# roatienza/efficientspeech

Measured on AMD Instinct MI355X. Metric: mel-frames/sec (whole node), full Phoneme2Mel forward, higher is better.
Workload: dtype f32 (weight GEMMs: fp32 operands split into 2 f16 pieces (22 significand bits, weights pre-scaled 2^8), 3 f16-MFMA products, fp32 accumulate)

## Files before the change

efficientspeech_amd/csrc/enc_block16.h:

```cpp
#pragma once
#include "chain16.h"
#include "enc_attn_ffn.h"

namespace esmi {

struct B016Lds {
    static constexpr int C = 32, LD = C + 4, NK = 128, LDX = NK + 4;
    static constexpr int xP = 0;
    static constexpr int xT = xP + 128 * LD;
    static constexpr int y1P = xT + C * LDX;
    static constexpr int priv = y1P + 130 * LD;
    static constexpr int priv_sz = 2 * 16 * LD;
    static constexpr int par = priv + 8 * priv_sz;
    static constexpr int wts = par + 512;
    static constexpr int total = wts + 24 * 256;
};
static_assert(B016Lds::total * 4 <= 160 * 1024, "enc_b0_16: LDS");
enum { B0_PROJB = 0, B0_LN1G = 32, B0_LN1B = 64, B0_FFNB = 96, B0_FFNB0 = 128, B0_FFNB2 = 160, B0_MLP2B = 192, B0_LN2G = 224, B0_LN2B = 256 };

template <int NKT>
__device__ __forceinline__ void enc_b0_16_body(const EncAttnFfnP& p) {
    using namespace c16;
    typedef B016Lds M;
    constexpr int C = M::C, LD = M::LD, LDX = M::LDX;
    ESMI_DYN_LDS(lds);
    ESMI_CT_INIT(0);
    ESMI_CT();
    const int nw = (int)(blockDim.x >> 6), w = uniform_i(wave_id());
    const int lane = lane_id(), i = lane & 15, g = lane >> 4;
    const int b = (int)blockIdx.x, rot = b;
    const int pos = 16 * w + i;
    unsigned* const ldu = reinterpret_cast<unsigned*>(lds);
    unsigned* const xP = ldu + M::xP;
    unsigned* const xT = ldu + M::xT;
    unsigned* const y1P = ldu + M::y1P;
    float* const xf = lds + M::priv + w * M::priv_sz;
    unsigned* const qP = ldu + M::priv + w * M::priv_sz + 16 * LD;
    float* const par = lds + M::par;
    float* const wM = lds + M::wts, * const wO = wM + 4 * 256, * const wF = wO + 4 * 256, * const w2 = wF + 12 * 256;
    const int wp = wpos(lane), lw1 = wlane(lane, 1);
    const f32x4 z4 = zero4();
    const int* idb = p.m.ids + (long)b * p.m.n_in;
    int id[3];
#pragma unroll
    for (int j = 0; j < 3; ++j) {
        const int ti = pos + j - 1;
        const bool ok = ti >= 0 && ti < p.m.n_in;
        const int v = idb[ok ? ti : 0];
        id[j] = !ok ? -1 : ((v < 0 || v >= p.m.vocab) ? 0 : v);
    }
    dma_frags(p.m.qkv_w, wM, 4, w, nw, lane, rot);
    dma_frags(p.proj_w, wO, 4, w, nw, lane, rot);
    dma_frags(p.ffn_w, wF, 12, w, nw, lane, rot);
    dma_frags(p.mlp2_w, w2, 4, w, nw, lane, rot);
    {
        const int v8 = lane >> 3, c8 = 4 * (lane & 7);
        auto pick8 = [&](const float* a0, const float* a1, const float* a2, const float* a3, const float* a4, const float* a5, const float* a6,
                         const float* a7) __attribute__((always_inline)) {
            const float* lo = v8 & 1 ? (v8 & 2 ? a3 : a1) : (v8 & 2 ? a2 : a0);
            const float* hi = v8 & 1 ? (v8 & 2 ? a7 : a5) : (v8 & 2 ? a6 : a4);
            return (v8 & 4 ? hi : lo) + c8;
        };
        if (w == 0 % nw) lds_dma16(pick8(p.proj_b, p.ln1_g, p.ln1_b, p.ffn_b, p.ffn_b0, p.ffn_b2, p.mlp2_b, p.ln2_g), par, lane);
        if (w == 1 % nw) lds_dma16(p.ln2_b + c8, par + B0_LN2B, lane);
    }
    if (w == 0 && lane < LD) {
        y1P[lane] = 0u;
        y1P[(16 * nw + 1) * LD + lane] = 0u;
    }
    if (nw < NKT) {
        for (int e = (int)threadIdx.x; e < C * LDX; e += (int)blockDim.x) xT[e] = 0u;
        for (int e = (int)threadIdx.x + 16 * nw * LD; e < 16 * NKT * LD; e += (int)blockDim.x) xP[e] = 0u;
        wg_sync_lds();
    }
    const bool rout = pos >= p.N;
    unsigned mb = 0;
    {
        const BufRsrc r_mask = make_rsrc(p.mask ? p.mask + (long)b * p.mask_len : nullptr, p.mask_len);
        for (int q = 0; q < p.mask_pool; ++q) {
            const int idx = pos * p.mask_pool + q;
            mb |= buf_ld_u8(r_mask, (unsigned)idx) | (unsigned)(p.mask && idx >= p.mask_len);
        }
    }
    const bool rz = !rout && mb != 0;
    ESMI_CT();
    f32x4 xacc[2] = {z4, z4};
#pragma unroll
    for (int j = 0; j < 3; ++j) {
        const float* row = p.m.emb_conv + ((long)j * p.m.vocab + (id[j] < 0 ? 0 : id[j])) * C + 4 * g;
#pragma unroll
        for (int nt = 0; nt < 2; ++nt) {
            const f32x4 v = ld4(row + 16 * nt);
            if (id[j] >= 0) xacc[nt] += v;
        }
    }
    if (rout) { xacc[0] = z4; xacc[1] = z4; }
#pragma unroll
    for (int nt = 0; nt < 2; ++nt) {
        planes_store(xP + pos * LD + wp, nt, C / 2, xacc[nt]);
        *reinterpret_cast<f32x4*>(xf + i * LD + 16 * nt + 4 * g) = xacc[nt];
    }
    lds_wave_sync();
#pragma unroll
    for (int ct = 0; ct < 2; ++ct) {
        f32x4 v;
#pragma unroll
        for (int r = 0; r < 4; ++r) v[r] = xf[(4 * g + r) * LD + 16 * ct + i];
        unsigned h1a, h2a, h1b, h2b;
        split_f16_pair(v[0], v[1], h1a, h2a);
        split_f16_pair(v[2], v[3], h1b, h2b);
        unsigned* dst = xT + (16 * ct + i) * LDX + 16 * (w >> 1) + 4 * g + 2 * (w & 1);
        *reinterpret_cast<u32x2*>(dst) = u32x2{h1a, h1b};
        *reinterpret_cast<u32x2*>(dst + M::NK / 2) = u32x2{h2a, h2b};
    }
    ESMI_CT();
    wait_vm0();
    wg_sync_lds();
    ESMI_CT();
    {
        f32x4 q[2] = {z4, z4};
        const unsigned* rowp = xP + pos * LD + 4 * g;
        gemm_pf<2, 1, 1>(q, wM, lw1, 0, [&](int) __attribute__((always_inline)) { return planes_load(rowp, 0, C / 2); });
#pragma unroll
        for (int nt = 0; nt < 2; ++nt) planes_store(qP + i * LD + wp, nt, C / 2, q[nt] * kF16WScaleInv);
        lds_wave_sync();
    }
    f32x4 s[NKT];
    {
        const f16x2p qf = planes_load(qP + i * LD + 4 * g, 0, C / 2);
        f16x2p kf[NKT];
#pragma unroll
        for (int kt = 0; kt < NKT; ++kt) kf[kt] = planes_load(xP + (16 * kt + i) * LD + 4 * g, 0, C / 2);
        sched_fence();
#pragma unroll
        for (int kt = 0; kt < NKT; ++kt) s[kt] = mfma16_f16(kf[kt].h2, qf.h1, z4);
#pragma unroll
        for (int kt = 0; kt < NKT; ++kt) s[kt] = mfma16_f16(kf[kt].h1, qf.h2, s[kt]);
#pragma unroll
        for (int kt = 0; kt < NKT; ++kt) s[kt] = mfma16_f16(kf[kt].h1, qf.h1, s[kt]);
    }
    ESMI_CT();
    float mx = -INFINITY;
#pragma unroll
    for (int kt = 0; kt < NKT; ++kt) {
#pragma unroll
        for (int r = 0; r < 4; ++r) {
            const int key = 16 * kt + 4 * g + r;
            const float v = key < p.N ? s[kt][r] * p.scale : -INFINITY;
            s[kt][r] = v;
            mx = fmaxf(mx, v);
        }
    }
    mx = row_max4(mx);
    float den = 0.0f;
#pragma unroll
    for (int kt = 0; kt < NKT; ++kt) {
#pragma unroll
        for (int r = 0; r < 4; ++r) {
            const float e = exp_fast_f32(s[kt][r] - mx);
            s[kt][r] = e;
            den += e;
        }
    }
    const float inv = rcp_fast_f32(row_sum4(den));
    ESMI_CT();
    f32x4 o[2] = {z4, z4};
    {
        f16x2p vf[NKT / 2][2];
#pragma unroll
        for (int ks = 0; ks < NKT / 2; ++ks) {
#pragma unroll
            for (int ct = 0; ct < 2; ++ct) {
                const unsigned* vp = xT + (16 * ct + i) * LDX + 16 * ks + 4 * g;
                vf[ks][ct].h1 = *reinterpret_cast<const u32x4*>(vp);
                vf[ks][ct].h2 = *reinterpret_cast<const u32x4*>(vp + M::NK / 2);
            }
        }
        sched_fence();
#pragma unroll
        for (int ks = 0; ks < NKT / 2; ++ks) {
            const f16x2p pf = split_f16x2(s[2 * ks] * inv, s[2 * ks + 1] * inv);
#pragma unroll
            for (int ct = 0; ct < 2; ++ct) o[ct] = mfma16_f16(vf[ks][ct].h2, pf.h1, o[ct]);
#pragma unroll
            for (int ct = 0; ct < 2; ++ct) o[ct] = mfma16_f16(vf[ks][ct].h1, pf.h2, o[ct]);
#pragma unroll
            for (int ct = 0; ct < 2; ++ct) o[ct] = mfma16_f16(vf[ks][ct].h1, pf.h1, o[ct]);
        }
    }
    ESMI_CT();
#pragma unroll
    for (int nt = 0; nt < 2; ++nt) planes_store(qP + i * LD + wp, nt, C / 2, o[nt]);
    lds_wave_sync();
    f32x4 y[2] = {z4, z4};
    {
        const unsigned* rowp = qP + i * LD + 4 * g;
        gemm_pf<2, 1, 1>(y, wO, lw1, 0, [&](int) __attribute__((always_inline)) { return planes_load(rowp, 0, C / 2); });
        f32x4 gg[2], bb[2];
#pragma unroll
        for (int nt = 0; nt < 2; ++nt) {
// ... 56 lines not shown
    }
    ESMI_CT();
}

template <int NKT>
__global__ __launch_bounds__(64 * 8, 2) void enc_b0_16_kernel(const EncAttnFfnP p) {
    enc_b0_16_body<NKT>(p);
}

struct B116Lds {
    static constexpr int C = 64, LD = C + 4, CIN = 32, NK = 64, LDX = NK + 4, LDC = 2 * C + 4;
    static constexpr int r1 = 0;
    static constexpr int r2 = r1 + 66 * LD;
    static constexpr int r3 = r2 + 64 * LD;
    static constexpr int r3_sz = 8 * 16 * LD;
    static constexpr int stats = r3 + r3_sz;
    static constexpr int par = stats + 256;
    static constexpr int wY = par + 768;
    static constexpr int wX = wY + 48 * 256;
    static constexpr int total = wX + 32 * 256;
};
static_assert(64 * B116Lds::LDC <= B116Lds::r3_sz && B116Lds::total * 4 <= 160 * 1024, "enc_b1_16: LDS");
enum { B1_PROJB = 0, B1_LN1G = 64, B1_LN1B = 128, B1_FFNB = 192, B1_FFNB0 = 256, B1_FFNB2 = 320, B1_MLP2B = 384, B1_LN2G = 448, B1_LN2B = 512 };

__device__ __forceinline__ void layernorm_pair16(f32x4 (&v)[2], const f32x4 (&gg)[2], const f32x4 (&bb)[2], float* st, int c, int i, int g,
                                                 float eps = 1e-5f) {
    using namespace c16;
    float s = (v[0][0] + v[0][1]) + (v[0][2] + v[0][3]) + ((v[1][0] + v[1][1]) + (v[1][2] + v[1][3]));
    const float mean_l = row_sum4(s) * (1.0f / 32.0f);
    float q = 0.0f;
#pragma unroll
    for (int nt = 0; nt < 2; ++nt) {
#pragma unroll
        for (int e = 0; e < 4; ++e) {
            const float d = v[nt][e] - mean_l;
            q = fmaf(d, d, q);
        }
    }
    const float m2_l = row_sum4(q);
    if (g == 0) *reinterpret_cast<f32x2*>(st + (c * 16 + i) * 2) = f32x2{mean_l, m2_l};
    wg_sync_lds();
    const f32x2 o = *reinterpret_cast<const f32x2*>(st + ((c ^ 1) * 16 + i) * 2);
    const float ma = c == 0 ? mean_l : o[0], mb = c == 0 ? o[0] : mean_l;
    const float qa = c == 0 ? m2_l : o[1], qb = c == 0 ? o[1] : m2_l;
    const float mean = 0.5f * (ma + mb);
    const float d = mb - ma;
    const float m2 = (qa + qb) + d * d * 16.0f;
    const float rstd = rsqrt_fast_f32(m2 * (1.0f / 64.0f) + eps);
#pragma unroll
    for (int nt = 0; nt < 2; ++nt) {
#pragma unroll
        for (int e = 0; e < 4; ++e) v[nt][e] = fmaf((v[nt][e] - mean) * rstd, gg[nt][e], bb[nt][e]);
    }
}

__device__ __forceinline__ void enc_b1_16_body(const EncAttnFfnP& p) {
    using namespace c16;
    typedef B116Lds M;
    constexpr int C = M::C, LD = M::LD, LDX = M::LDX, LDC = M::LDC, CIN = M::CIN, NKT = 4;
    ESMI_DYN_LDS(lds);
    ESMI_CT_INIT(1);
    ESMI_CT();
    const int nw = (int)(blockDim.x >> 6), w = uniform_i(wave_id());
    const int nrt = nw >> 1, rt = w >> 1, c = w & 1;
    const int lane = lane_id(), i = lane & 15, g = lane >> 4;
    const int b = (int)blockIdx.x, rot = b;
    const int pos = 16 * rt + i;
    unsigned* const ldu = reinterpret_cast<unsigned*>(lds);
    unsigned* const xP = ldu + M::r1;
    unsigned* const y1P = ldu + M::r1;
    unsigned* const xT = ldu + M::r2;
    unsigned* const hidP = ldu + M::r2;
    float* const xf = lds + M::r3 + w * (16 * LD);
    unsigned* const qP = ldu + M::r3 + w * (16 * LD);
    unsigned* const ctxP = ldu + M::r3;
    float* const st = lds + M::stats + rt * 64;
    float* const par = lds + M::par;
    float* const wY = lds + M::wY, * const wX = lds + M::wX;
    const int wp = wpos(lane), lw2 = wlane(lane, 2), lw4 = wlane(lane, 4);
    const f32x4 z4 = zero4();
    const bool rout = pos >= p.N;
    const BufRsrc r_in = make_rsrc(p.m.x_in + (long)b * p.m.n_in * CIN, (long)p.m.n_in * CIN * 4);
    const f16x2p a_in = global_bop(r_in, rout ? kBufOOB : (unsigned)(2 * pos * CIN * 4) + gl_lane(lane), 0);
    dma_frags(p.m.merge_w, wY, 8, w, nw, lane, rot);
    dma_frags(p.m.qkv_w, wY + 8 * 256, 32, w, nw, lane, rot);
    dma_frags(p.proj_w, wX, 32, w, nw, lane, rot);
    {
        const int v4 = lane >> 4, c4 = 4 * (lane & 15);
        auto pick4 = [&](const float* a0, const float* a1, const float* a2, const float* a3) __attribute__((always_inline)) {
            return (v4 & 2 ? (v4 & 1 ? a3 : a2) : (v4 & 1 ? a1 : a0)) + c4;
        };
        if (w == 0 % nw) lds_dma16(pick4(p.proj_b, p.ln1_g, p.ln1_b, p.ffn_b), par, lane);
        if (w == 1 % nw) lds_dma16(pick4(p.ffn_b0, p.ffn_b2, p.mlp2_b, p.ln2_g), par + 256, lane);
        if (w == 2 % nw) lds_dma16(p.ln2_b + c4, par + 512, lane);
    }
    if (nrt < NKT) {
        for (int e = (int)threadIdx.x; e < C * LDX; e += (int)blockDim.x) xT[e] = 0u;
        for (int e = (int)threadIdx.x + 16 * nrt * LD; e < 16 * NKT * LD; e += (int)blockDim.x) xP[e] = 0u;
        wg_sync_lds();
    }
    unsigned mb = 0;
    {
        const BufRsrc r_mask = make_rsrc(p.mask ? p.mask + (long)b * p.mask_len : nullptr, p.mask_len);
        for (int q = 0; q < p.mask_pool; ++q) {
            const int idx = pos * p.mask_pool + q;
            mb |= buf_ld_u8(r_mask, (unsigned)idx) | (unsigned)(p.mask && idx >= p.mask_len);
        }
    }
    const bool rz = !rout && mb != 0;
    wait_vm0();
    wg_sync_lds();
    ESMI_CT();
    f32x4 xh[2] = {z4, z4};
    gemm_pf<2, 2, 1>(xh, wY + c * 256, lw2, 0, [&](int) __attribute__((always_inline)) { return a_in; });
#pragma unroll
    for (int nt = 0; nt < 2; ++nt) {
        xh[nt] = rout ? z4 : xh[nt] * kF16WScaleInv;
        planes_store(xP + pos * LD + wp, 2 * c + nt, C / 2, xh[nt]);
        *reinterpret_cast<f32x4*>(xf + i * (CIN + 4) + 16 * nt + 4 * g) = xh[nt];
    }
    lds_wave_sync();
#pragma unroll
    for (int ct = 0; ct < 2; ++ct) {
        f32x4 v;
#pragma unroll
        for (int r = 0; r < 4; ++r) v[r] = xf[(4 * g + r) * (CIN + 4) + 16 * ct + i];
        unsigned h1a, h2a, h1b, h2b;
        split_f16_pair(v[0], v[1], h1a, h2a);
        split_f16_pair(v[2], v[3], h1b, h2b);
        unsigned* dst = xT + (32 * c + 16 * ct + i) * LDX + 16 * (rt >> 1) + 4 * g + 2 * (rt & 1);
        *reinterpret_cast<u32x2*>(dst) = u32x2{h1a, h1b};
        *reinterpret_cast<u32x2*>(dst + M::NK / 2) = u32x2{h2a, h2b};
    }
    wg_sync_lds();
    ESMI_CT();
    {
        f32x4 q[4] = {z4, z4, z4, z4};
        const unsigned* rowp = xP + pos * LD + 4 * g;
        gemm_pf<4, 4, 2>(q, wY + 8 * 256 + 2 * c * 256, lw4, 0, [&](int ks) __attribute__((always_inline)) { return planes_load(rowp, ks, C / 2); });
        lds_wave_sync();
#pragma unroll
        for (int nt = 0; nt < 4; ++nt) planes_store(qP + i * LD + wp, nt, C / 2, q[nt] * kF16WScaleInv);
        lds_wave_sync();
    }
    f32x4 s[NKT];
    {
        f16x2p qf[2], kf[2][NKT];
#pragma unroll
        for (int ks = 0; ks < 2; ++ks) {
            qf[ks] = planes_load(qP + i * LD + 4 * g, ks, C / 2);
#pragma unroll
            for (int kt = 0; kt < NKT; ++kt) kf[ks][kt] = planes_load(xP + (16 * kt + i) * LD + 4 * g, ks, C / 2);
        }
        sched_fence();
#pragma unroll
        for (int kt = 0; kt < NKT; ++kt) s[kt] = z4;
#pragma unroll
        for (int ks = 0; ks < 2; ++ks) {
#pragma unroll
            for (int kt = 0; kt < NKT; ++kt) s[kt] = mfma16_f16(kf[ks][kt].h2, qf[ks].h1, s[kt]);
#pragma unroll
            for (int kt = 0; kt < NKT; ++kt) s[kt] = mfma16_f16(kf[ks][kt].h1, qf[ks].h2, s[kt]);
#pragma unroll
            for (int kt = 0; kt < NKT; ++kt) s[kt] = mfma16_f16(kf[ks][kt].h1, qf[ks].h1, s[kt]);
        }
    }
    float mx = -INFINITY;
#pragma unroll
    for (int kt = 0; kt < NKT; ++kt) {
#pragma unroll
        for (int r = 0; r < 4; ++r) {
            const int key = 16 * kt + 4 * g + r;
            const float v = key < p.N ? s[kt][r] * p.scale : -INFINITY;
            s[kt][r] = v;
            mx = fmaxf(mx, v);
        }
    }
    mx = row_max4(mx);
    float den = 0.0f;
#pragma unroll
    for (int kt = 0; kt < NKT; ++kt) {
#pragma unroll
        for (int r = 0; r < 4; ++r) {
            const float e = exp_fast_f32(s[kt][r] - mx);
            s[kt][r] = e;
            den += e;
        }
    }
    const float inv = rcp_fast_f32(row_sum4(den));
    f32x4 o[4] = {z4, z4, z4, z4};
    {
        f16x2p vf[2][4];
#pragma unroll
        for (int ks = 0; ks < 2; ++ks) {
// ... 106 lines not shown
```

efficientspeech_amd/csrc/enc_va16.h:

```cpp
#pragma once
#include "chain16.h"
#include "enc_fuse_va.h"
#include "va_decide.h"

namespace esmi {

constexpr int kVa16MaxWaves = 8;
constexpr int kVa16Dim = 32;

struct Va16Lds {
    static constexpr int DIM = kVa16Dim;
    static constexpr int LDD = DIM + 4, LDT = 3 * DIM + 4, LDC = 2 * DIM + 4;
    static constexpr int ROWS = 16 * kVa16MaxWaves + 2;
    static constexpr int fused = 0;
    static constexpr int region = fused + ROWS * LDD;
    static constexpr int priv = 16 * LDC + 17 * LDD;
    static constexpr int region_sz = (ROWS * LDT > kVa16MaxWaves * priv ? ROWS * LDT : kVa16MaxWaves * priv);
    static constexpr int sdur = region + region_sz;
    static constexpr int par = sdur + 128;
    static constexpr int par_sz = 32 * 32 + 4 * 128;
    static constexpr int emb = par + par_sz;
    static constexpr int wA = emb + 2 * DIM * DIM;
    static constexpr int half = 9 * 1024;
    static constexpr int wB = wA + half;
    static constexpr int total = wB + half;
};
static_assert(Va16Lds::total * 4 <= 160 * 1024, "enc_va16: LDS");
inline int va16_lds_bytes() { return Va16Lds::total * (int)sizeof(float); }

enum { PV_MLPB0 = 0, PV_MLPB1 = 32, PV_UPB1 = 64, PV_FUSEB = 96, PV_LN2G = 128, PV_LN2B = 160, PV_EDGE = 192 ,
       PV_PRED = 256 ,
       PV_HEADB = 1024, PV_HEADG = PV_HEADB + 128, PV_HEADBE = PV_HEADG + 128 };

template <int KU>
__device__ __forceinline__ void enc_va16_body(const FuseVaP& p) {
    using namespace c16;
    typedef Va16Lds M;
    constexpr int DIM = M::DIM, LDD = M::LDD, LDT = M::LDT, LDC = M::LDC;
    static_assert((20 + 4 * KU) * 256 <= Va16Lds::half, "enc_va16: Fuse weights exceed an LDS half");
    ESMI_DYN_LDS(lds);
    ESMI_CT_INIT(2);
    ESMI_CT();
    const int nw = (int)(blockDim.x >> 6), w = uniform_i(wave_id());
    const int lane = lane_id(), i = lane & 15, g = lane >> 4;
    const int b = (int)blockIdx.x;
    const int r0 = 16 * w, pos = r0 + i;
    unsigned* const ldu = reinterpret_cast<unsigned*>(lds);
    unsigned* const fusedT = ldu + M::fused;
    unsigned* const hidT = ldu + M::region;
    unsigned* const catP = ldu + M::region + w * M::priv;
    unsigned* const tmpP = catP + 16 * LDC;
    int* const sdur = reinterpret_cast<int*>(lds + M::sdur);
    float* const par = lds + M::par;
    float* const embT = lds + M::emb;
    float* const wA = lds + M::wA;
    float* const wB = lds + M::wB;
    const int wp = wpos(lane);
    const int lw1 = wlane(lane, 1), lw4 = wlane(lane, 4);
    const f32x4 z4 = zero4();
    const int rot = (int)blockIdx.x;

    const bool rout = pos >= p.T;
    const BufRsrc r_mask = make_rsrc(p.mask ? p.mask + (long)b * p.T : nullptr, p.T);
    const bool rz = !rout && buf_ld_u8(r_mask, (unsigned)pos) != 0;
    const BufRsrc r_feat = make_rsrc(p.feat ? p.feat + (long)b * p.T * 4 * DIM : nullptr, (long)p.T * 4 * DIM * 4);
    const unsigned frow = rout ? kBufOOB : (unsigned)(pos * 4 * DIM * 4);
    const BufRsrc r_pt = make_rsrc(p.pitch_t ? p.pitch_t + (long)b * p.T : nullptr, (long)p.T * 4);
    const BufRsrc r_et = make_rsrc(p.energy_t ? p.energy_t + (long)b * p.T : nullptr, (long)p.T * 4);
    const BufRsrc r_dt = make_rsrc(p.dur_t ? p.dur_t + (long)b * p.T : nullptr, (long)p.T * 4);
    const unsigned trow = rout ? kBufOOB : (unsigned)(pos * 4);
    const float tv_p = buf_ld(r_pt, trow), tv_e = buf_ld(r_et, trow), tv_d = buf_ld(r_dt, trow);
    const float lb0 = p.pred[0].lin_b[0], lb1 = p.pred[1].lin_b[0], lb2 = p.pred[2].lin_b[0];
    const float sc_p = ctl_scale(p.pitch_s, b), sc_e = ctl_scale(p.energy_s, b), sc_d = ctl_scale(p.dur_s, b);
    const int e_i = (lane & 31) < DIM - 1 ? (lane & 31) : DIM - 2;
    const float edge_p = p.pred[0].bins[e_i], edge_e = p.pred[1].bins[e_i];
    const int n1 = p.n_i[1];
    const int n_base = floor_div(r0 - (KU - 1), 2);
    const int n_i = n_base + i;
    const BufRsrc r_f0 = make_rsrc(p.feats[0] + (long)b * p.n_i[0] * DIM, (long)p.n_i[0] * DIM * 4);
    const BufRsrc r_f1 = make_rsrc(p.feats[1] + (long)b * n1 * 2 * DIM, (long)n1 * 2 * DIM * 4);
    const unsigned o0 = rout ? kBufOOB : (unsigned)(pos * DIM * 4) + gl_lane(lane);
    const unsigned o1 = (n_i < 0 || n_i >= n1) ? kBufOOB : (unsigned)(n_i * 2 * DIM * 4) + gl_lane(lane);
    const f32x4 g0a = buf_ld4(r_f0, o0), g0b = buf_ld4(r_f0, o0 + 32u);
    const f32x4 g1a = buf_ld4(r_f1, o1), g1b = buf_ld4(r_f1, o1 + 32u), g1c = buf_ld4(r_f1, o1 + 128u), g1d = buf_ld4(r_f1, o1 + 160u);
    {
        dma_frags(p.mlp_w[0], wA, 4, w, nw, lane, rot);
        dma_frags(p.mlp_w[1], wA + 4 * 256, 8, w, nw, lane, rot);
        dma_frags(p.up_w[1], wA + 12 * 256, 4 * KU, w, nw, lane, rot);
        dma_frags(p.fuse_w, wA + (12 + 4 * KU) * 256, 8, w, nw, lane, rot);
        ESMI_CT();
        const int v8 = lane >> 3, c8 = 4 * (lane & 7);
        auto pick8 = [&](const float* a0, const float* a1, const float* a2, const float* a3, const float* a4, const float* a5, const float* a6,
                         const float* a7) __attribute__((always_inline)) {
            const float* lo = v8 & 1 ? (v8 & 2 ? a3 : a1) : (v8 & 2 ? a2 : a0);
            const float* hi = v8 & 1 ? (v8 & 2 ? a7 : a5) : (v8 & 2 ? a6 : a4);
            return (v8 & 4 ? hi : lo) + c8;
        };
        if (w == 0 % nw) lds_dma16(pick8(p.mlp_b[0], p.mlp_b[1], p.up_b[1], p.fuse_b, p.pred[2].ln2_g, p.pred[2].ln2_b, p.fuse_b, p.fuse_b), par, lane);
#pragma unroll
        for (int q = 0; q < 3; ++q) {
            const PredW& d = p.pred[q];
            if (w == (1 + q) % nw) lds_dma16(pick8(d.conv1_b, d.ln1_g, d.ln1_b, d.conv2_b, d.lin_w, d.lin_w, d.lin_w, d.lin_w), par + PV_PRED + 256 * q, lane);
        }
        if (p.h0) {
            if (w == 4 % nw) lds_dma16((lane < 32 ? p.head_b : p.head_g) + 4 * (lane & 31), par + PV_HEADB, lane);
            if (w == 5 % nw) lds_dma16(p.head_beta + 4 * (lane & 31), par + PV_HEADBE, lane);
        }
        if (w == 0) {
            if (lane < LDD) {
                fusedT[lane] = 0u;
                fusedT[(16 * nw + 1) * LDD + lane] = 0u;
            }
        }
        if (lane < LDD) tmpP[16 * LDD + lane] = 0u;
    }
    ESMI_CT();
    wait_vm0();
    ESMI_CT();
    wg_sync_lds();
    ESMI_CT();
    const f16x2p a0 = split_f16x2(g0a, g0b), a10 = split_f16x2(g1a, g1b), a11 = split_f16x2(g1c, g1d);
#pragma unroll
    for (int q = 0; q < 3; ++q) dma_frags(p.pred[q].conv1_w, wB + q * 12 * 256, 12, w, nw, lane, rot);
    dma_frags(p.pred[0].emb, embT, 4, w, nw, lane, rot);
    dma_frags(p.pred[1].emb, embT + DIM * DIM, 4, w, nw, lane, rot);
    if (w == 0) {
        const int l5 = lane & 31;
        par[PV_EDGE + lane] = l5 < DIM - 1 ? (lane < 32 ? edge_p : edge_e) : INFINITY;
    }
    f32x4 acc[2];
    {
        acc[0] = z4; acc[1] = z4;
        gemm_pf<2, 1, 1>(acc, wA, lw1, 0, [&](int) __attribute__((always_inline)) { return a0; });
#pragma unroll
        for (int nt = 0; nt < 2; ++nt) {
            const f32x4 bc = ld4_lds(par + PV_MLPB0 + 16 * nt + 4 * g);
            planes_store(catP + i * LDC + wp, nt, LDC / 2 - 2, fmaf4(acc[nt], kF16WScaleInv, bc));
        }
    }
    {
        acc[0] = z4; acc[1] = z4;
        gemm_pf<2, 1, 2>(acc, wA + 4 * 256, lw1, 0, [&](int ks) __attribute__((always_inline)) { return ks ? a11 : a10; });
        const bool n_ok = n_i >= 0 && n_i < n1;
#pragma unroll
        for (int nt = 0; nt < 2; ++nt) {
            const f32x4 bc = ld4_lds(par + PV_MLPB1 + 16 * nt + 4 * g);
            planes_store(tmpP + i * LDD + wp, nt, DIM / 2, n_ok ? fmaf4(acc[nt], kF16WScaleInv, bc) : z4);
        }
        lds_wave_sync();
        acc[0] = z4; acc[1] = z4;
        WFrags<2> uf[KU];
        f16x2p ua[KU];
#pragma unroll
        for (int j = 0; j < KU; ++j) {
            const int q = pos - j, nq = q >> 1;
            const bool ok = q >= 0 && (q & 1) == 0 && nq < n1;
            ua[j] = planes_load(tmpP + (ok ? nq - n_base : 16) * LDD + 4 * g, 0, DIM / 2);
            wfrags_load<2, 1, 2>(uf[j], 0, wA + (12 + 4 * j) * 256, lw1, 0);
        }
        sched_fence();
#pragma unroll
        for (int j = 0; j < KU; ++j) mma_all<2>(acc, uf[j], ua[j]);
#pragma unroll
        for (int nt = 0; nt < 2; ++nt) {
            const f32x4 bc = ld4_lds(par + PV_UPB1 + 16 * nt + 4 * g);
            planes_store(catP + i * LDC + wp, 2 + nt, LDC / 2 - 2, fmaf4(acc[nt], kF16WScaleInv, bc));
        }
        lds_wave_sync();
    }
    f32x4 fz[2];
    {
        acc[0] = z4; acc[1] = z4;
        const unsigned* rowp = catP + i * LDC + 4 * g;
        gemm_pf<2, 1, 2>(acc, wA + (12 + 4 * KU) * 256, lw1, 0, [&](int ks) __attribute__((always_inline)) { return planes_load(rowp, ks, LDC / 2 - 2); });
#pragma unroll
        for (int nt = 0; nt < 2; ++nt) {
            const f32x4 bc = ld4_lds(par + PV_FUSEB + 16 * nt + 4 * g);
            fz[nt] = (rout || rz) ? z4 : fmaf4(acc[nt], kF16WScaleInv, bc);
            planes_store(fusedT + (1 + pos) * LDD + wp, nt, DIM / 2, fz[nt]);
        }
    }
    ESMI_CT();
    wait_vm0();
    ESMI_CT();
    wg_sync_lds();
    ESMI_CT();
#pragma unroll
    for (int q = 0; q < 3; ++q) dma_frags(p.pred[q].conv2_w, wA + q * 12 * 256, 12, w, nw, lane, rot);
    if (w == 0) {
        for (int c = lane; c < LDT; c += 64) {
            hidT[c] = 0u;
            hidT[(16 * nw + 1) * LDT + c] = 0u;
        }
    }
    f32x4 c[6];
    {
#pragma unroll
        for (int n = 0; n < 6; ++n) c[n] = z4;
        const unsigned* rowp = fusedT + pos * LDD + 4 * g;
// ... 212 lines not shown
```

efficientspeech_amd/csrc/mel_decoder.h:

```cpp
#pragma once
#include <type_traits>

#include "dec_layout.h"

namespace esmi {

constexpr int kDecWps128 = 4, kDecWeightRing256 = 2;

__device__ __forceinline__ int batch_max_len(const int* __restrict__ mel_len, int B) {
    const int lane = lane_id();
    int v = 0;
    for (int j = lane; j < B; j += 64) v = max(v, mel_len[j]);
    float f = row_max32((float)v);
    f = fmaxf(f, swap32_f(f));
    return uniform_i((int)f);
}

template <int DX2, int NV>
__device__ __forceinline__ void dec_ln_regs(f32x4 (&v)[NV], const f32x4 (&g)[NV], const f32x4 (&be)[NV]) {
    float s = 0.0f;
#pragma unroll
    for (int k = 0; k < NV; ++k) s += (v[k][0] + v[k][1]) + (v[k][2] + v[k][3]);
    s = row_sum_n<16>(s);
    const float mean = s * (1.0f / DX2);
// ... 486 lines not shown
#pragma unroll
        for (int t = 0; t < NTW; ++t) {
            float* base = xs + opaque_i((kDecPadRows + 32 * MT * mh + i + shw) * LDSROW + ns * WCOLS + 32 * t + 4 * h);
            unsigned* pbase = reinterpret_cast<unsigned*>(xs) + opaque_i((kDecPadRows + 32 * MT * mh + i) * LDSROW + acc_col(t) / 2);
#pragma unroll
            for (int g = 0; g < 4; ++g) {
#pragma unroll
                for (int mt = 0; mt < MT; ++mt) {
                    f32x4 v;
#pragma unroll
                    for (int e = 0; e < 4; ++e) v[e] = inside[mt] ? acc[mt][t][4 * g + e] : 0.0f;
                    if (SPLIT && planes_) {
                        dec_store_planes<DX2>(pbase, 32 * mt * LDSROW + 4 * g, v);
                    } else if (keep_row[mt]) {
                        *reinterpret_cast<f32x4*>(base + 32 * mt * LDSROW + 8 * g) = v;
                    }
                }
            }
        }
    };
    auto ln_pass = [&](const float* pb0, bool block_end_, bool planes_, int shw) __attribute__((always_inline)) {
        const float* pb = pb0 + opaque_i(4 * ln_c);
        float* ln_ptr = owner_ptr();
        f32x4 g[NV], be[NV];
        dec_owner_ld(pb + P_G, g);
        dec_owner_ld(pb + P_B, be);
        f32x4 v[RPT][NV];
        owner_load(v, ln_ptr);
#pragma unroll
        for (int j = 0; j < RPT; ++j) dec_ln_regs<DX2>(v[j], g, be);
        if (block_end_) {
            dec_owner_ld(pb + P_SG, g);
            dec_owner_ld(pb + P_SB, be);
#pragma unroll
            for (int j = 0; j < RPT; ++j) {
#pragma unroll
                for (int k = 0; k < NV; ++k) v[j][k] += skip[j][k];
                dec_ln_regs<DX2>(v[j], g, be);
            }
        }
        if (edge_window) {
#pragma unroll
            for (int j = 0; j < RPT; ++j) {
#pragma unroll
                for (int k = 0; k < NV; ++k)
                    if (!row_inside(j)) v[j][k] = zero4();
            }
        }
        if (SPLIT && planes_) {
#pragma unroll
            for (int j = 0; j < RPT; ++j) {
#pragma unroll
                for (int k = 0; k < NV; ++k) {
                    typedef unsigned u32x2 __attribute__((ext_vector_type(2)));
                    unsigned h1a, h2a, h1b, h2b;
                    split_f16_pair(v[j][k][0], v[j][k][1], h1a, h2a);
                    split_f16_pair(v[j][k][2], v[j][k][3], h1b, h2b);
                    unsigned* rowp = reinterpret_cast<unsigned*>(ln_ptr + j * LDSROW) - 2 * ln_c + 2 * TPR * k;
                    *reinterpret_cast<u32x2*>(rowp) = u32x2{h1a, h1b};
                    *reinterpret_cast<u32x2*>(rowp + DX2 / 2) = u32x2{h2a, h2b};
                }
            }
            return;
        }
        float* wp = ln_ptr;
        if (STREAM && shw) {
            __syncthreads();
            wp = ln_ptr + shw * LDSROW;
        }
#pragma unroll
        for (int j = 0; j < RPT; ++j) {
            if (STREAM && ln_row0 + j + shw >= kDecRows) continue;
#pragma unroll
            for (int k = 0; k < NV; ++k) *reinterpret_cast<f32x4*>(wp + j * LDSROW + 4 * TPR * k) = v[j][k];
        }
    };
    typedef std::true_type TrueC;
    typedef std::false_type FalseC;
    constexpr int NTM = (SPLIT && DX2 > 128) ? 1 : NTW;
    typedef std::integral_constant<int, NTW> NtwC;
    typedef std::integral_constant<int, NTM> NtmC;

    if (p.h0) {
        static_assert(kDecRows * (DX2 / 4) % kDecThreads == 0, "whole passes");
        for (int it = 0; it < kDecRows * (DX2 / 4) / kDecThreads; ++it) {
            const int e = tid + it * kDecThreads;
            const int r = e / (DX2 / 4), q = e - r * (DX2 / 4);
            const int s = src[r];
            f32x4 v = zero4();
            if (s >= 0) v = STREAM ? __builtin_nontemporal_load(reinterpret_cast<const f32x4*>(p.h0 + (long)s * DX2 + 4 * q)) : ld4(p.h0 + (long)s * DX2 + 4 * q);
            else if (s == -2) {
                const f32x4 bb = *reinterpret_cast<const f32x4*>(pbuf + P_PWB + 4 * q);
#pragma unroll
                for (int c = 0; c < 4; ++c) v[c] = tanh_fast_f32(bb[c]);
            }
            *reinterpret_cast<f32x4*>(xs + (kDecPadRows + r) * LDSROW + 4 * q) = v;
        }
#ifdef ESMI_DEC_TRACE
        ESMI_STAMP_AT(54);
#endif
        __syncthreads();
#ifdef ESMI_DEC_TRACE
        ESMI_STAMP_AT(55);
#endif
        {
            const float* pb = pbuf + opaque_i(4 * ln_c);
            float* ln_ptr = owner_ptr();
            owner_load(skip, ln_ptr);
            unsigned pad_rows = 0;
#pragma unroll
            for (int j = 0; j < RPT; ++j) pad_rows |= (src[ln_row0 + j] == -2 ? 1u : 0u) << j;
            if (ballot64(pad_rows != 0u) != 0ull) {
                f32x4 g[NV], be[NV];
                dec_owner_ld(pb + P_G, g);
                dec_owner_ld(pb + P_B, be);
#pragma unroll
                for (int j = 0; j < RPT; ++j) {
                    f32x4 u[NV];
#pragma unroll
                    for (int k = 0; k < NV; ++k) u[k] = skip[j][k];
                    dec_ln_regs<DX2>(u, g, be);
#pragma unroll
                    for (int k = 0; k < NV; ++k) {
                        if ((pad_rows >> j) & 1u) skip[j][k] = u[k];
                        *reinterpret_cast<f32x4*>(ln_ptr + j * LDSROW + 4 * TPR * k) = skip[j][k];
                    }
                }
            }
        }
        carry_put(0);
        __syncthreads();
    } else {
        dec_zero_acc(acc);
        const int nchunks = p.d4 / 128;
        for (int ch = 0; ch < nchunks; ++ch) {
            if (ch > 0) __syncthreads();
            for (int e = tid; e < kDecRows * 32; e += kDecThreads) {
                const int r = e >> 5, q = e & 31;
                const int s = src[r];
                f32x4 v = zero4();
                if (s >= 0) v = ld4(p.x + (long)s * p.d4 + ch * 128 + 4 * q);
                *reinterpret_cast<f32x4*>(xs + (kDecPadRows + r) * LDSROW + 4 * q) = v;
            }
            __syncthreads();
#pragma unroll
            for (int k0 = 0; k0 < 16; k0 += KSUB) {
                load_b(wslice(0, ch), k0);
                mma_sub(0, k0);
            }
        }
        tanh_acc(pbuf + P_PWB);
        __syncthreads();
        store_acc();
        __syncthreads();
        {
            const float* pb = pbuf + opaque_i(4 * ln_c);
            float* ln_ptr = owner_ptr();
            f32x4 g[NV], be[NV];
            dec_owner_ld(pb + P_G, g);
            dec_owner_ld(pb + P_B, be);
#pragma unroll
            for (int j = 0; j < RPT; ++j) {
#pragma unroll
                for (int k = 0; k < NV; ++k) skip[j][k] = *reinterpret_cast<const f32x4*>(ln_ptr + j * LDSROW + 4 * TPR * k);
                dec_ln_regs<DX2>(skip[j], g, be);
#pragma unroll
                for (int k = 0; k < NV; ++k) {
                    if (!row_inside(j)) skip[j][k] = zero4();
                    *reinterpret_cast<f32x4*>(ln_ptr + j * LDSROW + 4 * TPR * k) = skip[j][k];
                }
            }
        }
        carry_put(0);
        __syncthreads();
    }

    ESMI_STAMP();
    int dw_cg = tid % CG, dw_r0 = (tid / CG) * RS;
    int blk = 0, lin = 0;
// ... 246 lines not shown
```

efficientspeech_amd/csrc/tu_enc_block16.hip:

```cpp
#include "launch.h"
#include "enc_block16.h"
#include "enc_va16.h"

using namespace esmi;
ESMI_TU_RANGE_SETTER(enc_block16)
ESMI_TU_CHAIN_TRACE_SETTER(enc_block16)

namespace esmi {

static bool b16_common_ok(const EncAttnFfnP& p) { return p.fold && p.N >= 1 && p.m.qkv_w && p.proj_w && p.ffn_w && p.mlp2_w; }
static bool b0_16_ok(const EncAttnFfnP& p) {
    return b16_common_ok(p) && p.C == 32 && p.h == 1 && p.m.k == 3 && p.m.stride == 1 && p.m.ids && p.m.emb_conv && p.N <= 128 && p.m.n_in == p.N;
}
static bool b1_16_ok(const EncAttnFfnP& p, int c_in) {
    return b16_common_ok(p) && p.C == 64 && p.h == 2 && p.m.k == 1 && p.m.stride == 2 && c_in == 32 && p.m.x_in && !p.m.ids && p.N <= 64 &&
           p.m.n_in >= 2 * p.N - 1;
}

#if ESMI_CHAIN_SPLIT
struct EncAll16P { EncAttnFfnP b0, b1; FuseVaP va; };
template <int NKT>
__global__ __launch_bounds__(64 * 8, 2) void enc_all16_kernel(const EncAll16P p) {
    enc_b0_16_body<NKT>(p.b0);
    wait_vm0();
    __syncthreads();
    enc_b1_16_body(p.b1);
    wait_vm0();
    __syncthreads();
    enc_va16_body<3>(p.va);
}
#endif

int launch_enc_all16(const EncAttnFfnP& b0, const EncAttnFfnP& b1, int c_in1, const FuseVaP& va, int dim, int kernel, hipStream_t st) {
#if ESMI_CHAIN_SPLIT
    if (!b0_16_ok(b0) || !b1_16_ok(b1, c_in1) || !enc_va16_ok(va, dim, kernel)) return ESMI_ERR_UNSUPPORTED;
    if (va.T != b0.N || b0.B != b1.B || b0.B != va.B) return ESMI_ERR_UNSUPPORTED;
    int nw = (b0.N + 15) / 16;
    const int nw1 = 2 * ((b1.N + 15) / 16);
    nw = (nw > nw1 ? nw : nw1);
    nw += nw & 1;
    if (nw > 8) return ESMI_ERR_UNSUPPORTED;
    EncAll16P q;
    q.b0 = b0; q.b1 = b1; q.va = va;
    int lds = B016Lds::total > B116Lds::total ? B016Lds::total : B116Lds::total;
    lds = (lds > Va16Lds::total ? lds : Va16Lds::total) * (int)sizeof(float);
#define ESMI_ALL(NKT) { ESMI_LAUNCH_LDS((enc_all16_kernel<NKT>), dim3(b0.B), dim3(64 * nw), lds, st, q); return launch_status(); }
    if (nw <= 2) ESMI_ALL(2)
    if (nw <= 4) ESMI_ALL(4)
    ESMI_ALL(8)
#undef ESMI_ALL
#else
    (void)b0; (void)b1; (void)c_in1; (void)va; (void)dim; (void)kernel; (void)st;
    return ESMI_ERR_UNSUPPORTED;
#endif
}

int launch_enc_block16(const EncAttnFfnP& p, int expansion, int c_in, hipStream_t st) {
#if ESMI_CHAIN_SPLIT
    if (expansion != 1) return ESMI_ERR_UNSUPPORTED;
    EncAttnFfnP q = p;
    q.wgs_per_b = 1; q.halo = 0;
    if (b0_16_ok(p)) {
        const int nw = (p.N + 15) / 16, lds = B016Lds::total * (int)sizeof(float);
#define ESMI_B0(NKT) { ESMI_LAUNCH_LDS((enc_b0_16_kernel<NKT>), dim3(p.B), dim3(64 * nw), lds, st, q); return launch_status(); }
        if (nw <= 2) ESMI_B0(2)
        if (nw <= 4) ESMI_B0(4)
        ESMI_B0(8)
#undef ESMI_B0
    }
    if (b1_16_ok(p, c_in)) {
        const int nrt = (p.N + 15) / 16, lds = B116Lds::total * (int)sizeof(float);
        ESMI_LAUNCH_LDS(enc_b1_16_kernel, dim3(p.B), dim3(128 * nrt), lds, st, q);
        return launch_status();
    }
    return ESMI_ERR_UNSUPPORTED;
#else
    (void)p; (void)expansion; (void)c_in; (void)st;
    return ESMI_ERR_UNSUPPORTED;
#endif
}

}
```

efficientspeech_amd/csrc/wavesim_shim.h:

```cpp
#pragma once

#ifdef ESMI_WAVESIM
#include "wavesim.h"
#define ESMI_DYN_LDS(name) float* name = (float*)wavesim::dyn_lds()
#define ESMI_LAUNCH(kern, grid, block, lds, stream, ...) \
    wavesim::launch(#kern, grid, block, lds, [&]() { kern(__VA_ARGS__); })
#else
#include <hip/hip_runtime.h>
#define ESMI_DYN_LDS(name) extern __shared__ __attribute__((aligned(16))) float name[]
#define ESMI_LAUNCH(kern, grid, block, lds, stream, ...) hipLaunchKernelGGL(kern, grid, block, lds, stream, __VA_ARGS__)
#endif

#include "esmi_types.h"

#ifndef ESMI_CHAIN_SPLIT
#define ESMI_CHAIN_SPLIT 1
#endif

namespace esmi {

#ifdef ESMI_WAVESIM
constexpr const char* kBackendName = "wavesim";
constexpr int kReduceGroups = 4;
constexpr int kLossBlocks = 8;
// ... 258 lines not shown
__device__ __forceinline__ float exp_fast_f32(float x) {
#ifdef ESMI_WAVESIM
    return exp2f(x * 1.4426950408889634f);
#else
    return __builtin_amdgcn_exp2f(x * 1.4426950408889634f);
#endif
}
__device__ __forceinline__ float rsqrt_fast_f32(float x) {
#ifdef ESMI_WAVESIM
    return 1.0f / sqrtf(x);
#else
    return __builtin_amdgcn_rsqf(x);
#endif
}
__device__ __forceinline__ float rcp_fast_f32(float x) {
#ifdef ESMI_WAVESIM
    return 1.0f / x;
#else
    return __builtin_amdgcn_rcpf(x);
#endif
}
__device__ __forceinline__ long long clock_shader() {
#ifdef ESMI_WAVESIM
    return 0;
#else
    return (long long)__builtin_amdgcn_s_memtime();
#endif
}
__device__ __forceinline__ long long clock_real100() {
#ifdef ESMI_WAVESIM
    return 0;
#else
    return (long long)__builtin_amdgcn_s_memrealtime();
#endif
}
__device__ __forceinline__ int opaque_i(int v) {
#ifndef ESMI_WAVESIM
    asm volatile("" : "+v"(v));
#endif
    return v;
}
__device__ __forceinline__ int uniform_i(int v) {
#ifdef ESMI_WAVESIM
    return v;
#else
    return __builtin_amdgcn_readfirstlane(v);
#endif
}
__device__ __forceinline__ float ctl_scale(const float* scale, int b) {
#ifdef ESMI_WAVESIM
    return scale ? scale[b] : 1.0f;
#else
    typedef const __attribute__((address_space(4))) float* const_f32_ptr;
    return scale ? *(const_f32_ptr)(scale + uniform_i(b)) : 1.0f;
#endif
}
__device__ __forceinline__ void lds_dma16(const void* gsrc_lane, void* lds_wave_base, int lane) {
#ifdef ESMI_WAVESIM
    reinterpret_cast<f32x4*>(lds_wave_base)[lane] = *reinterpret_cast<const f32x4*>(gsrc_lane);
#else
    (void)lane;
    __builtin_amdgcn_global_load_lds((const __attribute__((address_space(1))) void*)gsrc_lane,
                                     (__attribute__((address_space(3))) void*)lds_wave_base, 16, 0, 0);
#endif
}
constexpr unsigned kBufOOB = 0x80000000u;
#ifdef ESMI_WAVESIM
struct BufRsrc { const char* base; unsigned bytes; };
__device__ __forceinline__ BufRsrc make_rsrc(const void* p, long bytes) {
    BufRsrc r = {static_cast<const char*>(p), p ? (unsigned)(bytes < 0 ? 0 : (bytes > 0x7fffffffL ? 0x7fffffffL : bytes)) : 0u};
    return r;
}
__device__ __forceinline__ float buf_ld(const BufRsrc& r, unsigned off) {
    return (off < r.bytes && off + 4u <= r.bytes) ? *reinterpret_cast<const float*>(r.base + off) : 0.0f;
}
__device__ __forceinline__ f32x4 buf_ld4(const BufRsrc& r, unsigned off) {
    f32x4 z = {0.f, 0.f, 0.f, 0.f};
    return (off < r.bytes && off + 16u <= r.bytes) ? *reinterpret_cast<const f32x4*>(r.base + off) : z;
}
__device__ __forceinline__ unsigned buf_ld_u8(const BufRsrc& r, unsigned off) {
    return off < r.bytes ? (unsigned)*reinterpret_cast<const unsigned char*>(r.base + off) : 0u;
}
__device__ __forceinline__ f32x4 buf_ld4s(const BufRsrc& r, unsigned voff, unsigned soff) { return buf_ld4(r, voff + soff); }
__device__ __forceinline__ void buf_st(const BufRsrc& r, unsigned off, float v) {
    if (off < r.bytes && off + 4u <= r.bytes) *reinterpret_cast<float*>(const_cast<char*>(r.base) + off) = v;
}
__device__ __forceinline__ void buf_st_i(const BufRsrc& r, unsigned off, int v) {
    if (off < r.bytes && off + 4u <= r.bytes) *reinterpret_cast<int*>(const_cast<char*>(r.base) + off) = v;
}
__device__ __forceinline__ void buf_st_s(const BufRsrc& r, unsigned voff, unsigned soff, float v) { buf_st(r, voff == kBufOOB ? kBufOOB : voff + soff, v); }
__device__ __forceinline__ void buf_st4(const BufRsrc& r, unsigned off, const f32x4& v) {
    if (off < r.bytes && off + 16u <= r.bytes) *reinterpret_cast<f32x4*>(const_cast<char*>(r.base) + off) = v;
}
__device__ __forceinline__ void lds_wave_sync() { wavesim::shfl_i(0, 0); }
__device__ __forceinline__ void wait_vm0() {}
__device__ __forceinline__ void wg_sync_lds() { __syncthreads(); }
#else
typedef __amdgpu_buffer_rsrc_t BufRsrc;
__device__ __forceinline__ BufRsrc make_rsrc(const void* p, long bytes) {
    const int n = p ? (int)(bytes < 0 ? 0 : (bytes > 0x7fffffffL ? 0x7fffffffL : bytes)) : 0;
    return __builtin_amdgcn_make_buffer_rsrc(const_cast<void*>(p), 0, n, 0x00020000);
}
__device__ __forceinline__ float buf_ld(BufRsrc r, unsigned off) {
    return __builtin_bit_cast(float, __builtin_amdgcn_raw_buffer_load_b32(r, (int)off, 0, 0));
}
__device__ __forceinline__ f32x4 buf_ld4(BufRsrc r, unsigned off) {
    return __builtin_bit_cast(f32x4, __builtin_amdgcn_raw_buffer_load_b128(r, (int)off, 0, 0));
}
__device__ __forceinline__ unsigned buf_ld_u8(BufRsrc r, unsigned off) {
    return (unsigned)__builtin_amdgcn_raw_buffer_load_b8(r, (int)off, 0, 0);
}
__device__ __forceinline__ f32x4 buf_ld4s(BufRsrc r, unsigned voff, unsigned soff) {
    return __builtin_bit_cast(f32x4, __builtin_amdgcn_raw_buffer_load_b128(r, (int)voff, __builtin_amdgcn_readfirstlane((int)soff), 0));
}
__device__ __forceinline__ void buf_st(BufRsrc r, unsigned off, float v) {
    __builtin_amdgcn_raw_buffer_store_b32(__builtin_bit_cast(unsigned, v), r, (int)off, 0, 0);
}
__device__ __forceinline__ void buf_st_i(BufRsrc r, unsigned off, int v) {
    __builtin_amdgcn_raw_buffer_store_b32((unsigned)v, r, (int)off, 0, 0);
}
__device__ __forceinline__ void buf_st_s(BufRsrc r, unsigned voff, unsigned soff, float v) {
    __builtin_amdgcn_raw_buffer_store_b32(__builtin_bit_cast(unsigned, v), r, (int)voff, __builtin_amdgcn_readfirstlane((int)soff), 0);
}
__device__ __forceinline__ void buf_st4(BufRsrc r, unsigned off, const f32x4& v) {
    __builtin_amdgcn_raw_buffer_store_b128(__builtin_bit_cast(u32x4, v), r, (int)off, 0, 0);
}
__device__ __forceinline__ void wait_vm0() { asm volatile("s_waitcnt vmcnt(0)" ::: "memory"); }
__device__ __forceinline__ void wg_sync_lds() { asm volatile("s_waitcnt lgkmcnt(0)\n\ts_barrier" ::: "memory"); }
__device__ __forceinline__ void lds_wave_sync() { asm volatile("s_waitcnt lgkmcnt(0)" ::: "memory"); }
#endif

__device__ __forceinline__ void sched_fence() {
#ifndef ESMI_WAVESIM
    __builtin_amdgcn_sched_barrier(0);
#endif
}


inline int current_device() {
#ifdef ESMI_WAVESIM
    return 0;
#else
    int dev = 0;
    const hipError_t e = hipGetDevice(&dev);
    return e == hipSuccess ? dev : -(int)e;
#endif
}
inline int set_max_dynamic_lds(const void* fn, int bytes) {
#ifdef ESMI_WAVESIM
    (void)fn; (void)bytes;
    return 0;
#else
    return (int)hipFuncSetAttribute(fn, hipFuncAttributeMaxDynamicSharedMemorySize, bytes);
#endif
}
inline int read_device_flag(const int* dev_flag, hipStream_t stream, int* out) {
#ifdef ESMI_WAVESIM
    (void)stream;
    *out = *dev_flag;
    return 0;
#else
    hipError_t e = hipStreamSynchronize(stream);
    if (e == hipSuccess) e = hipMemcpy(out, dev_flag, sizeof(int), hipMemcpyDeviceToHost);
    return (int)e;
#endif
}
#if ESMI_RANGE_CHECK
static inline int store_range_flag_pointer(int* flag) {
#ifdef ESMI_WAVESIM
    g_esmi_range_flag = flag;
    return 0;
#else
    return (int)hipMemcpyToSymbol(HIP_SYMBOL(g_esmi_range_flag), &flag, sizeof(flag));
#endif
}
#endif

}
```

Before: 970.8 million.

## Hoist mask and embedding loads early and batch decoder h0 gathers via buffer loads

```diff
diff --git a/efficientspeech_amd/csrc/enc_block16.h b/efficientspeech_amd/csrc/enc_block16.h
--- a/efficientspeech_amd/csrc/enc_block16.h
+++ b/efficientspeech_amd/csrc/enc_block16.h
@@ -3,6 +3,24 @@
 #include "enc_attn_ffn.h"
 
 namespace esmi {
+
+constexpr int kMaskRegs = 4;
+struct MaskReq { unsigned byte[kMaskRegs]; unsigned beyond; };
+__device__ __forceinline__ MaskReq mask_request(const EncAttnFfnP& p, int b, int pos) {
+    MaskReq m;
+    const BufRsrc r_mask = make_rsrc(p.mask ? p.mask + (long)b * p.mask_len : nullptr, p.mask_len);
+    const int first = pos * p.mask_pool;
+#pragma unroll
+    for (int k = 0; k < kMaskRegs; ++k) m.byte[k] = buf_ld_u8(r_mask, k < p.mask_pool ? (unsigned)(first + k) : kBufOOB);
+    m.beyond = (unsigned)(p.mask && first + p.mask_pool > p.mask_len);
+    return m;
+}
+__device__ __forceinline__ bool mask_take(const MaskReq& m) {
+    unsigned mb = m.beyond;
+#pragma unroll
+    for (int k = 0; k < kMaskRegs; ++k) mb |= (unsigned)opaque_i((int)m.byte[k]);
+    return mb != 0;
+}
 
 struct B016Lds {
     static constexpr int C = 32, LD = C + 4, NK = 128, LDX = NK + 4;
@@ -49,6 +67,7 @@
         const int v = idb[ok ? ti : 0];
         id[j] = !ok ? -1 : ((v < 0 || v >= p.m.vocab) ? 0 : v);
     }
+    const MaskReq mreq = mask_request(p, b, pos);
     dma_frags(p.m.qkv_w, wM, 4, w, nw, lane, rot);
     dma_frags(p.proj_w, wO, 4, w, nw, lane, rot);
     dma_frags(p.ffn_w, wF, 12, w, nw, lane, rot);
@@ -74,24 +93,21 @@
         wg_sync_lds();
     }
     const bool rout = pos >= p.N;
-    unsigned mb = 0;
-    {
-        const BufRsrc r_mask = make_rsrc(p.mask ? p.mask + (long)b * p.mask_len : nullptr, p.mask_len);
-        for (int q = 0; q < p.mask_pool; ++q) {
-            const int idx = pos * p.mask_pool + q;
-            mb |= buf_ld_u8(r_mask, (unsigned)idx) | (unsigned)(p.mask && idx >= p.mask_len);
-        }
-    }
-    const bool rz = !rout && mb != 0;
     ESMI_CT();
     f32x4 xacc[2] = {z4, z4};
-#pragma unroll
-    for (int j = 0; j < 3; ++j) {
-        const float* row = p.m.emb_conv + ((long)j * p.m.vocab + (id[j] < 0 ? 0 : id[j])) * C + 4 * g;
-#pragma unroll
-        for (int nt = 0; nt < 2; ++nt) {
-            const f32x4 v = ld4(row + 16 * nt);
-            if (id[j] >= 0) xacc[nt] += v;
+    {
+        const BufRsrc r_emb = make_rsrc(p.m.emb_conv, (long)3 * p.m.vocab * C * 4);
+        f32x4 tv[3][2];
+#pragma unroll
+        for (int j = 0; j < 3; ++j) {
+            const unsigned off = id[j] < 0 ? kBufOOB : (unsigned)(((j * p.m.vocab + id[j]) * C + 4 * g) * 4);
+#pragma unroll
+            for (int nt = 0; nt < 2; ++nt) tv[j][nt] = buf_ld4(r_emb, off + 64u * nt);
+        }
+#pragma unroll
+        for (int j = 0; j < 3; ++j) {
+#pragma unroll
+            for (int nt = 0; nt < 2; ++nt) xacc[nt] += tv[j][nt];
         }
     }
     if (rout) { xacc[0] = z4; xacc[1] = z4; }
@@ -116,6 +132,7 @@
     ESMI_CT();
     wait_vm0();
     wg_sync_lds();
+    const bool rz = !rout && mask_take(mreq);
     ESMI_CT();
     {
         f32x4 q[2] = {z4, z4};
@@ -338,6 +355,7 @@
     const bool rout = pos >= p.N;
     const BufRsrc r_in = make_rsrc(p.m.x_in + (long)b * p.m.n_in * CIN, (long)p.m.n_in * CIN * 4);
     const f16x2p a_in = global_bop(r_in, rout ? kBufOOB : (unsigned)(2 * pos * CIN * 4) + gl_lane(lane), 0);
+    const MaskReq mreq = mask_request(p, b, pos);
     dma_frags(p.m.merge_w, wY, 8, w, nw, lane, rot);
     dma_frags(p.m.qkv_w, wY + 8 * 256, 32, w, nw, lane, rot);
     dma_frags(p.proj_w, wX, 32, w, nw, lane, rot);
@@ -355,17 +373,9 @@
         for (int e = (int)threadIdx.x + 16 * nrt * LD; e < 16 * NKT * LD; e += (int)blockDim.x) xP[e] = 0u;
         wg_sync_lds();
     }
-    unsigned mb = 0;
-    {
-        const BufRsrc r_mask = make_rsrc(p.mask ? p.mask + (long)b * p.mask_len : nullptr, p.mask_len);
-        for (int q = 0; q < p.mask_pool; ++q) {
-            const int idx = pos * p.mask_pool + q;
-            mb |= buf_ld_u8(r_mask, (unsigned)idx) | (unsigned)(p.mask && idx >= p.mask_len);
-        }
-    }
-    const bool rz = !rout && mb != 0;
     wait_vm0();
     wg_sync_lds();
+    const bool rz = !rout && mask_take(mreq);
     ESMI_CT();
     f32x4 xh[2] = {z4, z4};
     gemm_pf<2, 2, 1>(xh, wY + c * 256, lw2, 0, [&](int) __attribute__((always_inline)) { return a_in; });
diff --git a/efficientspeech_amd/csrc/enc_va16.h b/efficientspeech_amd/csrc/enc_va16.h
--- a/efficientspeech_amd/csrc/enc_va16.h
+++ b/efficientspeech_amd/csrc/enc_va16.h
@@ -32,7 +32,7 @@
        PV_PRED = 256 ,
        PV_HEADB = 1024, PV_HEADG = PV_HEADB + 128, PV_HEADBE = PV_HEADG + 128 };
 
-template <int KU>
+template <int KU, bool LATE_MASK = false>
 __device__ __forceinline__ void enc_va16_body(const FuseVaP& p) {
     using namespace c16;
     typedef Va16Lds M;
@@ -62,7 +62,10 @@
 
     const bool rout = pos >= p.T;
     const BufRsrc r_mask = make_rsrc(p.mask ? p.mask + (long)b * p.T : nullptr, p.T);
-    const bool rz = !rout && buf_ld_u8(r_mask, (unsigned)pos) != 0;
+    unsigned mbyte = 0;
+    bool rz = false;
+    if constexpr (LATE_MASK) mbyte = buf_ld_u8(r_mask, (unsigned)pos);
+    else rz = !rout && buf_ld_u8(r_mask, (unsigned)pos) != 0;
     const BufRsrc r_feat = make_rsrc(p.feat ? p.feat + (long)b * p.T * 4 * DIM : nullptr, (long)p.T * 4 * DIM * 4);
     const unsigned frow = rout ? kBufOOB : (unsigned)(pos * 4 * DIM * 4);
     const BufRsrc r_pt = make_rsrc(p.pitch_t ? p.pitch_t + (long)b * p.T : nullptr, (long)p.T * 4);
@@ -115,6 +118,7 @@
         if (lane < LDD) tmpP[16 * LDD + lane] = 0u;
     }
     ESMI_CT();
+    if constexpr (LATE_MASK) rz = !rout && mbyte != 0;
     wait_vm0();
     ESMI_CT();
     wg_sync_lds();
diff --git a/efficientspeech_amd/csrc/mel_decoder.h b/efficientspeech_amd/csrc/mel_decoder.h
--- a/efficientspeech_amd/csrc/mel_decoder.h
+++ b/efficientspeech_amd/csrc/mel_decoder.h
@@ -592,19 +592,34 @@
     typedef std::integral_constant<int, NTM> NtmC;
 
     if (p.h0) {
-        static_assert(kDecRows * (DX2 / 4) % kDecThreads == 0, "whole passes");
-        for (int it = 0; it < kDecRows * (DX2 / 4) / kDecThreads; ++it) {
-            const int e = tid + it * kDecThreads;
-            const int r = e / (DX2 / 4), q = e - r * (DX2 / 4);
-            const int s = src[r];
-            f32x4 v = zero4();
-            if (s >= 0) v = STREAM ? __builtin_nontemporal_load(reinterpret_cast<const f32x4*>(p.h0 + (long)s * DX2 + 4 * q)) : ld4(p.h0 + (long)s * DX2 + 4 * q);
-            else if (s == -2) {
-                const f32x4 bb = *reinterpret_cast<const f32x4*>(pbuf + P_PWB + 4 * q);
-#pragma unroll
-                for (int c = 0; c < 4; ++c) v[c] = tanh_fast_f32(bb[c]);
-            }
-            *reinterpret_cast<f32x4*>(xs + (kDecPadRows + r) * LDSROW + 4 * q) = v;
+        constexpr int NIT = kDecRows * (DX2 / 4) / kDecThreads, NBAT = NIT < 8 ? NIT : 8;
+        static_assert(kDecRows * (DX2 / 4) % kDecThreads == 0 && NIT % NBAT == 0, "whole passes, whole batches");
+        const int h0_rows = p.cum ? p.T : L, s_base = b * h0_rows;
+        const BufRsrc r_h0 = make_rsrc(p.h0 + (long)s_base * DX2, (long)h0_rows * DX2 * 4);
+        for (int it0 = 0; it0 < NIT; it0 += NBAT) {
+            int sv[NBAT];
+            f32x4 hv[NBAT];
+#pragma unroll
+            for (int k = 0; k < NBAT; ++k) sv[k] = src[(tid + (it0 + k) * kDecThreads) / (DX2 / 4)];
+#pragma unroll
+            for (int k = 0; k < NBAT; ++k) {
+                const int e = tid + (it0 + k) * kDecThreads;
+                const int q = e % (DX2 / 4);
+                const unsigned off = sv[k] >= 0 ? (unsigned)(((sv[k] - s_base) * DX2 + 4 * q) * 4) : kBufOOB;
+                hv[k] = STREAM ? buf_ld4_nt(r_h0, off) : buf_ld4(r_h0, off);
+            }
+#pragma unroll
+            for (int k = 0; k < NBAT; ++k) {
+                const int e = tid + (it0 + k) * kDecThreads;
+                const int r = e / (DX2 / 4), q = e - r * (DX2 / 4);
+                f32x4 v = hv[k];
+                if (sv[k] == -2) {
+                    const f32x4 bb = *reinterpret_cast<const f32x4*>(pbuf + P_PWB + 4 * q);
+#pragma unroll
+                    for (int c = 0; c < 4; ++c) v[c] = tanh_fast_f32(bb[c]);
+                }
+                *reinterpret_cast<f32x4*>(xs + (kDecPadRows + r) * LDSROW + 4 * q) = v;
+            }
         }
 #ifdef ESMI_DEC_TRACE
         ESMI_STAMP_AT(54);
diff --git a/efficientspeech_amd/csrc/tu_enc_block16.hip b/efficientspeech_amd/csrc/tu_enc_block16.hip
--- a/efficientspeech_amd/csrc/tu_enc_block16.hip
+++ b/efficientspeech_amd/csrc/tu_enc_block16.hip
@@ -8,7 +8,9 @@
 
 namespace esmi {
 
-static bool b16_common_ok(const EncAttnFfnP& p) { return p.fold && p.N >= 1 && p.m.qkv_w && p.proj_w && p.ffn_w && p.mlp2_w; }
+static bool b16_common_ok(const EncAttnFfnP& p) {
+    return p.fold && p.N >= 1 && p.m.qkv_w && p.proj_w && p.ffn_w && p.mlp2_w && p.mask_pool <= kMaskRegs;
+}
 static bool b0_16_ok(const EncAttnFfnP& p) {
     return b16_common_ok(p) && p.C == 32 && p.h == 1 && p.m.k == 3 && p.m.stride == 1 && p.m.ids && p.m.emb_conv && p.N <= 128 && p.m.n_in == p.N;
 }
@@ -19,15 +21,32 @@
 
 #if ESMI_CHAIN_SPLIT
 struct EncAll16P { EncAttnFfnP b0, b1; FuseVaP va; };
+template <typename T>
+__device__ __forceinline__ T kernarg_member(const EncAll16P& p, size_t off) {
+#ifdef ESMI_WAVESIM
+    return *reinterpret_cast<const T*>(reinterpret_cast<const char*>(&p) + off);
+#else
+    (void)p;
+    typedef const __attribute__((address_space(4))) char* KernargPtr;
+    unsigned long long a = (unsigned long long)(KernargPtr)__builtin_amdgcn_kernarg_segment_ptr();
+    int lo = (int)(unsigned)a, hi = (int)(unsigned)(a >> 32);
+    asm volatile("" : "+s"(lo), "+s"(hi));
+    a = (unsigned long long)(unsigned)uniform_i(lo) | ((unsigned long long)(unsigned)uniform_i(hi) << 32);
+    typedef const __attribute__((address_space(4))) T* MemberPtr;
+    T v;
+    __builtin_memcpy(&v, (MemberPtr)(a + off), sizeof(T));
+    return v;
+#endif
+}
 template <int NKT>
 __global__ __launch_bounds__(64 * 8, 2) void enc_all16_kernel(const EncAll16P p) {
     enc_b0_16_body<NKT>(p.b0);
     wait_vm0();
     __syncthreads();
-    enc_b1_16_body(p.b1);
+    enc_b1_16_body(kernarg_member<EncAttnFfnP>(p, offsetof(EncAll16P, b1)));
     wait_vm0();
     __syncthreads();
-    enc_va16_body<3>(p.va);
+    enc_va16_body<3, true>(kernarg_member<FuseVaP>(p, offsetof(EncAll16P, va)));
 }
 #endif
 
diff --git a/efficientspeech_amd/csrc/wavesim_shim.h b/efficientspeech_amd/csrc/wavesim_shim.h
--- a/efficientspeech_amd/csrc/wavesim_shim.h
+++ b/efficientspeech_amd/csrc/wavesim_shim.h
@@ -364,6 +364,7 @@
     return off < r.bytes ? (unsigned)*reinterpret_cast<const unsigned char*>(r.base + off) : 0u;
 }
 __device__ __forceinline__ f32x4 buf_ld4s(const BufRsrc& r, unsigned voff, unsigned soff) { return buf_ld4(r, voff + soff); }
+__device__ __forceinline__ f32x4 buf_ld4_nt(const BufRsrc& r, unsigned off) { return buf_ld4(r, off); }
 __device__ __forceinline__ void buf_st(const BufRsrc& r, unsigned off, float v) {
     if (off < r.bytes && off + 4u <= r.bytes) *reinterpret_cast<float*>(const_cast<char*>(r.base) + off) = v;
 }
@@ -395,6 +396,9 @@
 __device__ __forceinline__ f32x4 buf_ld4s(BufRsrc r, unsigned voff, unsigned soff) {
     return __builtin_bit_cast(f32x4, __builtin_amdgcn_raw_buffer_load_b128(r, (int)voff, __builtin_amdgcn_readfirstlane((int)soff), 0));
 }
+__device__ __forceinline__ f32x4 buf_ld4_nt(BufRsrc r, unsigned off) {
+    return __builtin_bit_cast(f32x4, __builtin_amdgcn_raw_buffer_load_b128(r, (int)off, 0, 2));
+}
 __device__ __forceinline__ void buf_st(BufRsrc r, unsigned off, float v) {
     __builtin_amdgcn_raw_buffer_store_b32(__builtin_bit_cast(unsigned, v), r, (int)off, 0, 0);
 }
```

Result: slower. 949.0 million (-2.3%).
